# helmholtz-analytics/mpi4torch

Hardware: AMD Instinct MI355X
Metric: allreduce_fwdbwd_algbw_GBps (higher is better)
Workload: dtype bf16; 1 GPU; model=allreduce_1GiB_bf16_fwd_bwd, parallelism=dp1

## Files before the change

csrc/common.hpp:

```cpp
#pragma once

#include <torch/types.h>
#include <c10/util/Exception.h>

#include <cstdint>
#include <string>

namespace m4a {

enum RedOp : int64_t {
  kMax = 0,
  kMin = 1,
  kSum = 2,
  kProd = 3,
  kLAnd = 4,
  kBAnd = 5,
  kLOr = 6,
  kBOr = 7,
  kLXor = 8,
  kBXor = 9,
  kMinLoc = 10,
  kMaxLoc = 11,
};

inline const char* red_op_name(int64_t op) {
  switch (op) {
    case kMax: return "MPI_MAX";
    case kMin: return "MPI_MIN";
    case kSum: return "MPI_SUM";
    case kProd: return "MPI_PROD";
    case kLAnd: return "MPI_LAND";
    case kBAnd: return "MPI_BAND";
    case kLOr: return "MPI_LOR";
    case kBOr: return "MPI_BOR";
    case kLXor: return "MPI_LXOR";
    case kBXor: return "MPI_BXOR";
    case kMinLoc: return "MPI_MINLOC";
    case kMaxLoc: return "MPI_MAXLOC";
    default: return "<invalid op>";
  }
}

struct Config {
  bool force_host_staging = false;
  bool trace_enabled = false;
  bool debug_collectives = false;
  bool force_full_path = false;
  int64_t op_timeout_ms = 0;
  bool force_hierarchical = false;
  int64_t pipeline_chunk_bytes = 256ll << 20;
  enum AllreduceEngine : int { kAllreduceAuto = 0, kAllreduceNative, kAllreduceRccl };
  int allreduce_engine = kAllreduceAuto;
};

Config& config();
void reload_config_from_env();

}
```

csrc/extension.cpp:

```cpp

#include "ops.hpp"
#include "transport.hpp"

#include <torch/script.h>
#include <torch/extension.h>

#include <rccl/rccl.h>

namespace m4a {
namespace {

std::string& world_group_name() {
  static std::string name;
  return name;
}

c10::intrusive_ptr<Communicator> comm_world() {
  return c10::make_intrusive<Communicator>(world_group_name());
}

c10::intrusive_ptr<Communicator> comm_from_group(std::string group_name) {
  return c10::make_intrusive<Communicator>(std::move(group_name));
}

// ... 42 lines not shown
  m.def("JoinDummies", join_dummies_op);
}

}
}

PYBIND11_MODULE(TORCH_EXTENSION_NAME, m) {
  m.doc() = "mpi4torch_amd native core: RCCL-over-xGMI autograd collectives";

  m.def("_set_world_group_name",
        [](const std::string& name) { m4a::world_group_name() = name; });
  m.def("_get_world_group_name",
        []() { return m4a::world_group_name(); });

  m.def("force_host_staging",
        [](bool enabled) { m4a::config().force_host_staging = enabled; });
  m.def("host_staging_forced",
        []() { return m4a::config().force_host_staging; });

  m.def("force_full_path",
        [](bool enabled) { m4a::config().force_full_path = enabled; });

  m.def("_pack_roundtrip", &m4a::debug_pack_roundtrip);
  m.def("_bitwise_reduce", &m4a::debug_bitwise_reduce);
  m.def("_fp8_reduce", &m4a::debug_fp8_reduce);
  m.def("_arith_reduce", &m4a::debug_arith_reduce);
  m.def("_pairloc_reduce", &m4a::debug_pairloc_reduce);
  m.def("_mx8_quantize", &m4a::debug_mx8_quantize);
  m.def("_mx8_reduce", &m4a::debug_mx8_reduce);
  m.def("_mx8_dequantize", &m4a::debug_mx8_dequantize, py::arg("payload"),
        py::arg("scales"), py::arg("numel"), py::arg("dtype"),
        py::arg("out") = c10::optional<at::Tensor>());
  m.def("reload_config", &m4a::reload_config_from_env);

  m.def("_rccl_version", []() {
    int v = 0;
    ncclGetVersion(&v);
    return v;
  });

  m.attr("MPI_MAX") = (int64_t)m4a::kMax;
  m.attr("MPI_MIN") = (int64_t)m4a::kMin;
  m.attr("MPI_SUM") = (int64_t)m4a::kSum;
  m.attr("MPI_PROD") = (int64_t)m4a::kProd;
  m.attr("MPI_LAND") = (int64_t)m4a::kLAnd;
  m.attr("MPI_BAND") = (int64_t)m4a::kBAnd;
  m.attr("MPI_LOR") = (int64_t)m4a::kLOr;
  m.attr("MPI_BOR") = (int64_t)m4a::kBOr;
  m.attr("MPI_LXOR") = (int64_t)m4a::kLXor;
  m.attr("MPI_BXOR") = (int64_t)m4a::kBXor;
  m.attr("MPI_MINLOC") = (int64_t)m4a::kMinLoc;
  m.attr("MPI_MAXLOC") = (int64_t)m4a::kMaxLoc;
}
```

csrc/kernels.hip:

```cpp

#include <hip/hip_runtime.h>
#include <hip/hip_fp8.h>
#include "kernels.hpp"

namespace m4a {

namespace {

struct SlabArgs {
  const char* src;
  char* dst;
  long long row_b;
  long long chunks_per_row;
  long long total_chunks;
  long long src_pitch_b;
  long long dst_pitch_b;
};

template <int N>
struct SlabPack {
  SlabArgs s[N];
};

typedef unsigned int v4u __attribute__((ext_vector_type(4)));
template <typename T>
struct NtVec {
  using type = T;
};
template <>
struct NtVec<uint4> {
  using type = v4u;
};

template <typename VecT, int NSLABS>
__global__ __launch_bounds__(256) void slab_copy_kernel(SlabPack<NSLABS> pack) {
  constexpr long long G = (long long)sizeof(VecT);
  const SlabArgs& a = pack.s[blockIdx.z];
  const long long stride = (long long)gridDim.x * blockDim.x;
  for (long long i = (long long)blockIdx.x * blockDim.x + threadIdx.x;
       i < a.total_chunks; i += stride) {
    const long long b = i / a.chunks_per_row;
    const long long c = i - b * a.chunks_per_row;
    const char* srow = a.src + b * a.src_pitch_b;
    char* drow = a.dst + b * a.dst_pitch_b;
    long long head =
        (G - ((long long)(uintptr_t)drow & (G - 1))) & (G - 1);
    if (head > a.row_b) head = a.row_b;
    const long long body = (a.row_b - head) / G;
    if (c < body) {
      using NT = typename NtVec<VecT>::type;
      const NT* sp = reinterpret_cast<const NT*>(srow + head) + c;
      NT* dp = reinterpret_cast<NT*>(drow + head) + c;
      __builtin_nontemporal_store(__builtin_nontemporal_load(sp), dp);
    } else {
      for (long long k = 0; k < head; ++k) drow[k] = srow[k];
      for (long long k = head + body * G; k < a.row_b; ++k) drow[k] = srow[k];
    }
  }
}

template <typename VecT>
void launch_bucket(const SlabDesc* descs, int n, hipStream_t stream) {
  constexpr long long G = (long long)sizeof(VecT);
  while (n > 0) {
    const int take = n < kMaxSlabsPerLaunch ? n : kMaxSlabsPerLaunch;
    SlabPack<kMaxSlabsPerLaunch> pack{};
    long long max_chunks = 0;
    for (int i = 0; i < take; ++i) {
      const SlabDesc& d = descs[i];
      SlabArgs& a = pack.s[i];
      a.src = static_cast<const char*>(d.src);
      a.dst = static_cast<char*>(d.dst);
      a.row_b = d.count * d.after_b;
      a.src_pitch_b = d.src_pitch_b;
      a.dst_pitch_b = d.dst_pitch_b;
      a.chunks_per_row = (a.row_b >= G ? a.row_b / G : 0) + 1;
      a.total_chunks = d.before * a.chunks_per_row;
      if (a.total_chunks > max_chunks) max_chunks = a.total_chunks;
    }
    for (int i = take; i < kMaxSlabsPerLaunch; ++i) {
      pack.s[i] = pack.s[0];
      pack.s[i].total_chunks = 0;
    }
    if (max_chunks > 0) {
      long long blocks = (max_chunks + 255) / 256;
      if (blocks > 4096) blocks = 4096;
      if (blocks < 1) blocks = 1;
      dim3 grid((unsigned)blocks, 1, (unsigned)take);
      hipLaunchKernelGGL((slab_copy_kernel<VecT, kMaxSlabsPerLaunch>), grid,
                         dim3(256), 0, stream, pack);
    }
    descs += take;
    n -= take;
  }
}


template <int Q>
__device__ inline uint4 byte_window_q(const unsigned int d[8], int rbits) {
  if (rbits == 0) return make_uint4(d[Q], d[Q + 1], d[Q + 2], d[Q + 3]);
  auto take = [&](int j) {
    unsigned long long w =
        ((unsigned long long)d[Q + j + 1] << 32) | d[Q + j];
    return (unsigned int)(w >> rbits);
  };
  return make_uint4(take(0), take(1), take(2), take(3));
}

__device__ inline uint4 byte_window(const uint4& lo, const uint4& hi, int s) {
  const unsigned int d[8] = {lo.x, lo.y, lo.z, lo.w, hi.x, hi.y, hi.z, hi.w};
  const int q = s >> 2;
  const int rbits = (s & 3) * 8;
  switch (q) {
    case 0: return byte_window_q<0>(d, rbits);
    case 1: return byte_window_q<1>(d, rbits);
    case 2: return byte_window_q<2>(d, rbits);
    default: return byte_window_q<3>(d, rbits);
  }
}

template <int NSLABS>
__global__ __launch_bounds__(256) void slab_copy_shift_kernel(
    SlabPack<NSLABS> pack) {
  const SlabArgs& a = pack.s[blockIdx.z];
  const long long stride = (long long)gridDim.x * blockDim.x;
  for (long long i = (long long)blockIdx.x * blockDim.x + threadIdx.x;
       i < a.total_chunks; i += stride) {
    const long long b = i / a.chunks_per_row;
    const long long c = i - b * a.chunks_per_row;
    const char* srow = a.src + b * a.src_pitch_b;
    char* drow = a.dst + b * a.dst_pitch_b;
    long long head = (16 - ((long long)(uintptr_t)drow & 15)) & 15;
    if (head > a.row_b) head = a.row_b;
    const long long body = (a.row_b - head) / 16;
    const char* sbase = srow + head;
    const int s = (int)((uintptr_t)sbase & 15);
    const long long bodyv = (s == 0) ? body : (body > 0 ? body - 1 : 0);
    const long long vs = (s == 0 || s <= head) ? 0 : 1;
    if (c >= vs && c < bodyv) {
      const char* sal = sbase - s + 16 * c;
      if (s == 0) {
        __builtin_nontemporal_store(
            __builtin_nontemporal_load(reinterpret_cast<const v4u*>(sal)),
            reinterpret_cast<v4u*>(drow + head + 16 * c));
      } else {
        const uint4 lo = *reinterpret_cast<const uint4*>(sal);
        const uint4 hi = *reinterpret_cast<const uint4*>(sal + 16);
        const uint4 w = byte_window(lo, hi, s);
        __builtin_nontemporal_store(
            *reinterpret_cast<const v4u*>(&w),
            reinterpret_cast<v4u*>(drow + head + 16 * c));
      }
    } else if (c == bodyv) {
      if (bodyv <= vs) {
        for (long long k = 0; k < a.row_b; ++k) drow[k] = srow[k];
      } else {
        const long long lo_end = head + vs * 16;
        for (long long k = 0; k < lo_end; ++k) drow[k] = srow[k];
        for (long long k = head + bodyv * 16; k < a.row_b; ++k) {
          drow[k] = srow[k];
        }
      }
    }
  }
}

void launch_shift_bucket(const SlabDesc* descs, int n, hipStream_t stream) {
  while (n > 0) {
    const int take = n < kMaxSlabsPerLaunch ? n : kMaxSlabsPerLaunch;
    SlabPack<kMaxSlabsPerLaunch> pack{};
    long long max_chunks = 0;
    for (int i = 0; i < take; ++i) {
      const SlabDesc& d = descs[i];
      SlabArgs& a = pack.s[i];
      a.src = static_cast<const char*>(d.src);
      a.dst = static_cast<char*>(d.dst);
      a.row_b = d.count * d.after_b;
      a.src_pitch_b = d.src_pitch_b;
      a.dst_pitch_b = d.dst_pitch_b;
      a.chunks_per_row = (a.row_b >= 16 ? a.row_b / 16 : 0) + 1;
      a.total_chunks = d.before * a.chunks_per_row;
      if (a.total_chunks > max_chunks) max_chunks = a.total_chunks;
    }
    for (int i = take; i < kMaxSlabsPerLaunch; ++i) {
      pack.s[i] = pack.s[0];
      pack.s[i].total_chunks = 0;
    }
    if (max_chunks > 0) {
      long long blocks = (max_chunks + 255) / 256;
      if (blocks > 4096) blocks = 4096;
      if (blocks < 1) blocks = 1;
      dim3 grid((unsigned)blocks, 1, (unsigned)take);
      hipLaunchKernelGGL((slab_copy_shift_kernel<kMaxSlabsPerLaunch>), grid,
                         dim3(256), 0, stream, pack);
    }
    descs += take;
    n -= take;
  }
}

inline int slab_granule(const SlabDesc& d) {
  const long long delta =
      (long long)((uintptr_t)d.src - (uintptr_t)d.dst);
  const long long pdelta = d.src_pitch_b - d.dst_pitch_b;
  for (int g = 16; g > 1; g >>= 1) {
    if ((delta & (g - 1)) == 0 && (pdelta & (g - 1)) == 0) return g;
  }
  return 1;
}

struct OpAnd {
  __device__ static uint4 apply(uint4 a, uint4 b) {
    return make_uint4(a.x & b.x, a.y & b.y, a.z & b.z, a.w & b.w);
  }
  __device__ static unsigned char apply(unsigned char a, unsigned char b) {
    return a & b;
  }
};
struct OpOr {
  __device__ static uint4 apply(uint4 a, uint4 b) {
    return make_uint4(a.x | b.x, a.y | b.y, a.z | b.z, a.w | b.w);
  }
  __device__ static unsigned char apply(unsigned char a, unsigned char b) {
    return a | b;
  }
};
struct OpXor {
  __device__ static uint4 apply(uint4 a, uint4 b) {
    return make_uint4(a.x ^ b.x, a.y ^ b.y, a.z ^ b.z, a.w ^ b.w);
  }
  __device__ static unsigned char apply(unsigned char a, unsigned char b) {
    return a ^ b;
  }
};

template <typename T, typename Op>
__global__ __launch_bounds__(256) void bitwise_reduce_kernel(
    const T* __restrict__ in, T* __restrict__ out, long long chunk_elems,
    long long nranks) {
  using NT = typename NtVec<T>::type;
  const long long stride = (long long)gridDim.x * blockDim.x;
  for (long long i = (long long)blockIdx.x * blockDim.x + threadIdx.x;
       i < chunk_elems; i += stride) {
    NT av = __builtin_nontemporal_load(reinterpret_cast<const NT*>(in) + i);
    T acc = *reinterpret_cast<const T*>(&av);
    for (long long r = 1; r < nranks; ++r) {
      NT bv = __builtin_nontemporal_load(reinterpret_cast<const NT*>(in) +
                                         r * chunk_elems + i);
      acc = Op::apply(acc, *reinterpret_cast<const T*>(&bv));
    }
    __builtin_nontemporal_store(*reinterpret_cast<const NT*>(&acc),
                                reinterpret_cast<NT*>(out) + i);
  }
}

template <typename T, typename Op>
void launch_bitred(const void* in, void* out, int64_t chunk_elems, int nranks,
                   hipStream_t stream) {
  long long blocks = (chunk_elems + 255) / 256;
  if (blocks > 4096) blocks = 4096;
  if (blocks < 1) blocks = 1;
  hipLaunchKernelGGL((bitwise_reduce_kernel<T, Op>), dim3((unsigned)blocks),
                     dim3(256), 0, stream, static_cast<const T*>(in),
                     static_cast<T*>(out), (long long)chunk_elems,
                     (long long)nranks);
}

}

void launch_slab_copy(const SlabDesc* descs, int n, hipStream_t stream) {
  int i = 0;
  while (i < n) {
    const int g = slab_granule(descs[i]);
    int j = i + 1;
    while (j < n && slab_granule(descs[j]) == g) ++j;
    switch (g) {
      case 16: launch_bucket<uint4>(descs + i, j - i, stream); break;
      case 8: launch_bucket<unsigned long long>(descs + i, j - i, stream); break;
      case 4: launch_bucket<unsigned int>(descs + i, j - i, stream); break;
      default:
        launch_shift_bucket(descs + i, j - i, stream);
        break;
    }
    i = j;
  }
}

void launch_bitwise_reduce(const void* in, void* out, int64_t chunk_bytes,
                           int nranks, int op, hipStream_t stream) {
  const bool vec16 = (chunk_bytes % 16 == 0) &&
                     (reinterpret_cast<uintptr_t>(in) % 16 == 0) &&
                     (reinterpret_cast<uintptr_t>(out) % 16 == 0);
  if (vec16) {
    const int64_t elems = chunk_bytes / 16;
    switch (op) {
// ... 85 lines not shown
    for (int d = 0; d < 4; ++d) {
      unsigned int od = 0;
      for (int k = 0; k < 4; ++k) {
        od |= (unsigned int)f32_to_fp8<E5M2>(acc[4 * d + k]) << (8 * k);
      }
      o[d] = od;
    }
    __builtin_nontemporal_store(o, reinterpret_cast<v4u*>(out) + i);
  }
}

template <typename Op, bool E5M2>
__global__ __launch_bounds__(256) void fp8_reduce_kernel_scalar(
    const unsigned char* __restrict__ in, unsigned char* __restrict__ out,
    long long n, long long nranks) {
  const long long stride = (long long)gridDim.x * blockDim.x;
  for (long long i = (long long)blockIdx.x * blockDim.x + threadIdx.x;
       i < n; i += stride) {
    float acc = fp8_to_f32<E5M2>(in[i]);
    for (long long r = 1; r < nranks; ++r) {
      acc = Op::apply(acc, fp8_to_f32<E5M2>(in[r * n + i]));
    }
    out[i] = f32_to_fp8<E5M2>(acc);
  }
}

template <typename Op, bool E5M2>
void launch_fp8_reduce_t(const void* in, void* out, int64_t n, int nranks,
                         hipStream_t stream) {
  const bool vec = (n % 16 == 0) &&
                   (reinterpret_cast<uintptr_t>(in) % 16 == 0) &&
                   (reinterpret_cast<uintptr_t>(out) % 16 == 0);
  const long long work = vec ? n / 16 : n;
  long long blocks = (work + 255) / 256;
  if (blocks > 4096) blocks = 4096;
  if (blocks < 1) blocks = 1;
  if (vec) {
    hipLaunchKernelGGL((fp8_reduce_kernel<Op, E5M2>), dim3((unsigned)blocks),
                       dim3(256), 0, stream,
                       static_cast<const unsigned char*>(in),
                       static_cast<unsigned char*>(out), (long long)n,
                       (long long)nranks);
  } else {
    hipLaunchKernelGGL((fp8_reduce_kernel_scalar<Op, E5M2>),
                       dim3((unsigned)blocks), dim3(256), 0, stream,
                       static_cast<const unsigned char*>(in),
                       static_cast<unsigned char*>(out), (long long)n,
                       (long long)nranks);
  }
}

}

void launch_fp8_reduce(const void* in, void* out, int64_t n_elems, int nranks,
                       int op, bool e5m2, hipStream_t stream) {
  auto dispatch = [&](auto opv) {
    using Op = decltype(opv);
    if (e5m2) {
      launch_fp8_reduce_t<Op, true>(in, out, n_elems, nranks, stream);
    } else {
      launch_fp8_reduce_t<Op, false>(in, out, n_elems, nranks, stream);
    }
  };
  switch (op) {
    case 0: dispatch(FAdd{}); break;
    case 1: dispatch(FMul{}); break;
    case 2: dispatch(FMin{}); break;
    default: dispatch(FMax{}); break;
  }
}


namespace {

constexpr long long kMaxGrid = 1ll << 30;

struct TF32 {
  using S = float;
  static constexpr int E = 4;
  __device__ static void unpack(v4u w, float* f) {
    for (int d = 0; d < 4; ++d) f[d] = __uint_as_float(w[d]);
  }
  __device__ static v4u pack(const float* f) {
    v4u o;
    for (int d = 0; d < 4; ++d) o[d] = __float_as_uint(f[d]);
    return o;
  }
  __device__ static float ld(const S* p) { return *p; }
  __device__ static void st(S* p, float f) { *p = f; }
};

__device__ inline unsigned int f32_to_bf16_bits(float f) {
  const unsigned int u = __float_as_uint(f);
  if (f != f) return 0x7FC0u;
  return (u + 0x7FFFu + ((u >> 16) & 1u)) >> 16;
}

struct TBF16 {
  using S = unsigned short;
  static constexpr int E = 8;
  __device__ static void unpack(v4u w, float* f) {
    for (int d = 0; d < 4; ++d) {
      f[2 * d] = __uint_as_float(w[d] << 16);
      f[2 * d + 1] = __uint_as_float(w[d] & 0xFFFF0000u);
    }
  }
  __device__ static v4u pack(const float* f) {
    v4u o;
// ... 86 lines not shown
      arith_reduce_scalar_range<T, Op>(own, staged, stride_b, nranks, me, out,
                                       nvec * E, n_elems, 1);
    }
  }
}

template <typename T, typename Op>
__global__ __launch_bounds__(256) void arith_reduce_kernel_scalar(
    const char* __restrict__ own, const char* __restrict__ staged,
    long long stride_b, int nranks, int me, char* __restrict__ out,
    long long n_elems) {
  arith_reduce_scalar_range<T, Op>(
      own, staged, stride_b, nranks, me, out,
      (long long)blockIdx.x * blockDim.x + threadIdx.x, n_elems,
      (long long)gridDim.x * blockDim.x);
}

__global__ __launch_bounds__(256) void arith_reduce_copy_kernel(
    const char* __restrict__ src, char* __restrict__ dst, long long nvec,
    long long nbytes) {
  const long long items = nvec + (nbytes > nvec * 16 ? 1 : 0);
  for (long long t = blockIdx.x; t * 256 < items; t += gridDim.x) {
    const long long i = t * 256 + threadIdx.x;
    if (i < nvec) {
      __builtin_nontemporal_store(
          __builtin_nontemporal_load(reinterpret_cast<const v4u*>(src) + i),
          reinterpret_cast<v4u*>(dst) + i);
    } else if (i == nvec) {
      for (long long k = nvec * 16; k < nbytes; ++k) dst[k] = src[k];
    }
  }
}

inline unsigned arith_grid(long long items) {
  long long blocks = (items + 255) / 256;
  if (blocks > kMaxGrid) blocks = kMaxGrid;
  if (blocks < 1) blocks = 1;
  return (unsigned)blocks;
}

template <typename T, typename Op>
void launch_arith_reduce_t(const void* own, const void* staged,
                           int64_t stride_elems, int nranks, int me,
                           void* out, int64_t n, hipStream_t stream) {
  const long long esize = (long long)sizeof(typename T::S);
  const long long stride_b = (long long)stride_elems * esize;
  auto al16 = [](const void* p) {
    return reinterpret_cast<uintptr_t>(p) % 16 == 0;
  };
  const bool vec = al16(own) && al16(out) && al16(staged) && stride_b % 16 == 0;
  if (vec) {
    const long long nvec = n / T::E;
    const long long items = nvec + (n % T::E ? 1 : 0);
    hipLaunchKernelGGL((arith_reduce_kernel<T, Op>), dim3(arith_grid(items)),
                       dim3(256), 0, stream, static_cast<const char*>(own),
                       static_cast<const char*>(staged), stride_b, nranks, me,
                       static_cast<char*>(out), nvec, (long long)n);
  } else {
    hipLaunchKernelGGL((arith_reduce_kernel_scalar<T, Op>),
                       dim3(arith_grid(n)), dim3(256), 0, stream,
                       static_cast<const char*>(own),
                       static_cast<const char*>(staged), stride_b, nranks, me,
                       static_cast<char*>(out), (long long)n);
  }
}

}

void launch_arith_copy(const void* src, void* dst, int64_t nbytes,
                       hipStream_t stream) {
  if (nbytes <= 0) return;
  if (reinterpret_cast<uintptr_t>(src) % 16 != 0 ||
      reinterpret_cast<uintptr_t>(dst) % 16 != 0) {
    SlabDesc d;
    d.src = src;
    d.dst = dst;
    d.before = 1;
    d.count = 1;
    d.after_b = nbytes;
    d.src_pitch_b = nbytes;
    d.dst_pitch_b = nbytes;
    launch_slab_copy(&d, 1, stream);
    return;
  }
  const long long nvec = nbytes / 16;
  const long long items = nvec + (nbytes % 16 ? 1 : 0);
  hipLaunchKernelGGL(arith_reduce_copy_kernel, dim3(arith_grid(items)),
                     dim3(256), 0, stream, static_cast<const char*>(src),
                     static_cast<char*>(dst), nvec, (long long)nbytes);
}

void launch_arith_reduce(const void* own, const void* staged,
                         int64_t stride_elems, int nranks, int me, void* out,
                         int64_t n_elems, int op, int dtype,
                         hipStream_t stream) {
  if (n_elems <= 0) return;
  if (nranks == 1) {
    launch_arith_copy(own, out, n_elems * (dtype == 0 ? 4 : 2), stream);
    return;
  }
  auto dispatch = [&](auto opv) {
    using Op = decltype(opv);
    switch (dtype) {
      case 0:
        launch_arith_reduce_t<TF32, Op>(own, staged, stride_elems, nranks, me,
                                        out, n_elems, stream);
        break;
      case 1:
        launch_arith_reduce_t<TBF16, Op>(own, staged, stride_elems, nranks, me,
                                         out, n_elems, stream);
        break;
      default:
        launch_arith_reduce_t<TF16, Op>(own, staged, stride_elems, nranks, me,
                                        out, n_elems, stream);
        break;
    }
  };
  switch (op) {
    case 0: dispatch(FAdd{}); break;
    case 1: dispatch(FMul{}); break;
    case 2: dispatch(FMin{}); break;
    default: dispatch(FMax{}); break;
  }
}


#include <hip/hip_fp16.h>
#include <hip/hip_bfloat16.h>

namespace {

// ... 6 lines not shown
template <>
__device__ inline bool pl_lt<hip_bfloat16>(hip_bfloat16 a, hip_bfloat16 b) {
  return (float)a < (float)b;
}
template <typename T>
__device__ inline bool pl_eq(T a, T b) { return !pl_lt(a, b) && !pl_lt(b, a); }

template <typename T, bool MAXLOC>
__global__ __launch_bounds__(256) void pairloc_reduce_kernel(
    const T* __restrict__ in, T* __restrict__ out, long long n,
    long long nranks) {
  const long long stride = (long long)gridDim.x * blockDim.x;
  for (long long i = (long long)blockIdx.x * blockDim.x + threadIdx.x;
       i < n; i += stride) {
    T bv = in[2 * i];
    T bl = in[2 * i + 1];
    for (long long r = 1; r < nranks; ++r) {
      const T v = in[r * 2 * n + 2 * i];
      const T l = in[r * 2 * n + 2 * i + 1];
      const bool better = MAXLOC ? pl_lt(bv, v) : pl_lt(v, bv);
      if (better || (pl_eq(v, bv) && pl_lt(l, bl))) {
        bv = v;
        bl = l;
      }
    }
    out[2 * i] = bv;
    out[2 * i + 1] = bl;
  }
}

template <typename T>
void launch_pairloc_t(const void* in, void* out, int64_t n, int nranks,
                      int op, hipStream_t stream) {
  long long blocks = (n + 255) / 256;
  if (blocks > 4096) blocks = 4096;
  if (blocks < 1) blocks = 1;
  if (op == 0) {
    hipLaunchKernelGGL((pairloc_reduce_kernel<T, false>),
                       dim3((unsigned)blocks), dim3(256), 0, stream,
                       static_cast<const T*>(in), static_cast<T*>(out),
                       (long long)n, (long long)nranks);
  } else {
    hipLaunchKernelGGL((pairloc_reduce_kernel<T, true>),
                       dim3((unsigned)blocks), dim3(256), 0, stream,
                       static_cast<const T*>(in), static_cast<T*>(out),
                       (long long)n, (long long)nranks);
  }
}

}

void launch_pairloc_reduce(const void* in, void* out, int64_t n_pairs,
                           int nranks, int op, int dtype,
                           hipStream_t stream) {
  switch (dtype) {
    case 0: launch_pairloc_t<float>(in, out, n_pairs, nranks, op, stream); break;
    case 1: launch_pairloc_t<double>(in, out, n_pairs, nranks, op, stream); break;
    case 2: launch_pairloc_t<__half>(in, out, n_pairs, nranks, op, stream); break;
    case 3: launch_pairloc_t<hip_bfloat16>(in, out, n_pairs, nranks, op, stream); break;
    case 4: launch_pairloc_t<signed char>(in, out, n_pairs, nranks, op, stream); break;
    case 5: launch_pairloc_t<unsigned char>(in, out, n_pairs, nranks, op, stream); break;
    case 6: launch_pairloc_t<short>(in, out, n_pairs, nranks, op, stream); break;
    case 7: launch_pairloc_t<int>(in, out, n_pairs, nranks, op, stream); break;
    default: launch_pairloc_t<long long>(in, out, n_pairs, nranks, op, stream); break;
  }
}

}
```

csrc/kernels.hpp:

```cpp
#pragma once

#include <hip/hip_runtime_api.h>
#include <cstdint>

namespace m4a {

struct SlabDesc {
  const void* src;
  void* dst;
  int64_t before;
  int64_t count;
  int64_t after_b;
  int64_t src_pitch_b;
  int64_t dst_pitch_b;
};

constexpr int kMaxSlabsPerLaunch = 8;

void launch_slab_copy(const SlabDesc* descs, int n, hipStream_t stream);

void launch_bitwise_reduce(const void* in, void* out, int64_t chunk_bytes,
                           int nranks, int op, hipStream_t stream);

void launch_pairloc_reduce(const void* in, void* out, int64_t n_pairs,
                           int nranks, int op, int dtype, hipStream_t stream);

void launch_fp8_reduce(const void* in, void* out, int64_t n_elems,
                       int nranks, int op, bool e5m2, hipStream_t stream);

void launch_arith_reduce(const void* own, const void* staged,
                         int64_t stride_elems, int nranks, int me, void* out,
                         int64_t n_elems, int op, int dtype,
                         hipStream_t stream);
void launch_arith_copy(const void* src, void* dst, int64_t nbytes,
                       hipStream_t stream);

void launch_mx8_quantize(const void* in, void* payload, void* scales,
                         int64_t n_elems, int dtype, hipStream_t stream);
void launch_mx8_reduce(const void* payload_in, const void* scales_in,
                       void* payload_out, void* scales_out, int64_t n_groups,
                       int nranks, hipStream_t stream);
void launch_mx8_dequantize(const void* payload, const void* scales, void* out,
                           int64_t n_elems, int dtype, hipStream_t stream);

}
```

csrc/mx8_kernels.hip:

```cpp

#include <hip/hip_runtime.h>
#include <hip/hip_fp8.h>
#include "kernels.hpp"

namespace m4a {

namespace {

typedef unsigned int v4u __attribute__((ext_vector_type(4)));
typedef unsigned int v2u __attribute__((ext_vector_type(2)));
typedef unsigned char u8;

constexpr unsigned kInfBits = 0x7f800000u;
constexpr unsigned kQNaNBits = 0x7fc00000u;

enum { kF32 = 0, kBF16 = 1, kF16 = 2 };

template <int K> struct Elem { using type = float; };
template <> struct Elem<kBF16> { using type = unsigned short; };
template <> struct Elem<kF16> { using type = unsigned short; };

__device__ inline float e4m3_to_f32(u8 b) {
  __hip_fp8_e4m3 v;
  v.__x = b;
// ... 336 lines not shown
      w[0] = t[0];
      w[EPL / 4 - 1] = t[1];
    }
    float x[EPL];
    for (int d = 0; d < EPL / 4; ++d) {
      for (int k = 0; k < 4; ++k) {
        x[4 * d + k] = mx8_dequant((u8)(w[d] >> (8 * k)), sb);
      }
    }
    __builtin_nontemporal_store(pack16<K, EPL>(x),
                                reinterpret_cast<v4u*>(out) + i);
  }
  const int tail = (int)(N - nfull * 32);
  if (tail > 0 && blockIdx.x == gridDim.x - 1 && threadIdx.x == 0) {
    dequant_group_scalar<K>(pay + nfull * 32, sc[nfull], tail,
                            reinterpret_cast<T*>(out) + nfull * 32);
  }
}

template <int K>
__global__ __launch_bounds__(256) void mx8_dequantize_kernel_scalar(
    const u8* __restrict__ pay, const u8* __restrict__ sc,
    void* __restrict__ out, long long G, long long N) {
  using T = typename Elem<K>::type;
  const long long stride = (long long)gridDim.x * blockDim.x;
  for (long long g = (long long)blockIdx.x * blockDim.x + threadIdx.x; g < G;
       g += stride) {
    const long long left = N - g * 32;
    dequant_group_scalar<K>(pay + g * 32, sc[g], left < 32 ? (int)left : 32,
                            reinterpret_cast<T*>(out) + g * 32);
  }
}

inline unsigned grid_for(long long work) {
  long long blocks = (work + 255) / 256;
  if (blocks > 4096) blocks = 4096;
  if (blocks < 1) blocks = 1;
  return (unsigned)blocks;
}

inline bool aligned(const void* p, uintptr_t a) {
  return (reinterpret_cast<uintptr_t>(p) & (a - 1)) == 0;
}

template <int K>
void launch_quantize_t(const void* in, void* pay, void* sc, int64_t N,
                       hipStream_t stream) {
  constexpr int LPG = K == kF32 ? 8 : 4;
  const long long G = (N + 31) / 32;
  const long long nfull = N / 32;
  if (aligned(in, 16) && aligned(pay, 32 / LPG)) {
    hipLaunchKernelGGL((mx8_quantize_kernel<K>), dim3(grid_for(nfull * LPG)),
                       dim3(256), 0, stream, in, static_cast<u8*>(pay),
                       static_cast<u8*>(sc), nfull, (long long)N);
  } else {
    hipLaunchKernelGGL((mx8_quantize_kernel_scalar<K>), dim3(grid_for(G)),
                       dim3(256), 0, stream, in, static_cast<u8*>(pay),
                       static_cast<u8*>(sc), G, (long long)N);
  }
}

template <int K>
void launch_dequantize_t(const void* pay, const void* sc, void* out, int64_t N,
                         hipStream_t stream) {
  constexpr int LPG = K == kF32 ? 8 : 4;
  const long long G = (N + 31) / 32;
  const long long nfull = N / 32;
  if (aligned(out, 16) && aligned(pay, 32 / LPG)) {
    hipLaunchKernelGGL((mx8_dequantize_kernel<K>),
                       dim3(grid_for(nfull * LPG)), dim3(256), 0, stream,
                       static_cast<const u8*>(pay),
                       static_cast<const u8*>(sc), out, nfull, (long long)N);
  } else {
    hipLaunchKernelGGL((mx8_dequantize_kernel_scalar<K>), dim3(grid_for(G)),
                       dim3(256), 0, stream, static_cast<const u8*>(pay),
                       static_cast<const u8*>(sc), out, G, (long long)N);
  }
}

}

void launch_mx8_quantize(const void* in, void* payload, void* scales,
                         int64_t n_elems, int dtype, hipStream_t stream) {
  if (n_elems <= 0) return;
  switch (dtype) {
    case 0: launch_quantize_t<kF32>(in, payload, scales, n_elems, stream); break;
    case 1: launch_quantize_t<kBF16>(in, payload, scales, n_elems, stream); break;
    default: launch_quantize_t<kF16>(in, payload, scales, n_elems, stream); break;
  }
}

void launch_mx8_reduce(const void* payload_in, const void* scales_in,
                       void* payload_out, void* scales_out, int64_t n_groups,
                       int nranks, hipStream_t stream) {
  if (n_groups <= 0) return;
  const u8* pin = static_cast<const u8*>(payload_in);
  const u8* sin = static_cast<const u8*>(scales_in);
  u8* pout = static_cast<u8*>(payload_out);
  u8* sout = static_cast<u8*>(scales_out);
  if (aligned(pin, 16) && aligned(pout, 16)) {
    hipLaunchKernelGGL(mx8_reduce_kernel, dim3(grid_for(n_groups * 2)),
                       dim3(256), 0, stream, pin, sin, pout, sout,
                       (long long)n_groups, (long long)nranks);
  } else {
    hipLaunchKernelGGL(mx8_reduce_kernel_scalar, dim3(grid_for(n_groups)),
                       dim3(256), 0, stream, pin, sin, pout, sout,
                       (long long)n_groups, (long long)nranks);
  }
}

void launch_mx8_dequantize(const void* payload, const void* scales, void* out,
                           int64_t n_elems, int dtype, hipStream_t stream) {
  if (n_elems <= 0) return;
  switch (dtype) {
    case 0: launch_dequantize_t<kF32>(payload, scales, out, n_elems, stream); break;
    case 1: launch_dequantize_t<kBF16>(payload, scales, out, n_elems, stream); break;
    default: launch_dequantize_t<kF16>(payload, scales, out, n_elems, stream); break;
  }
}

}
```

csrc/ops.cpp:

```cpp

#include "ops.hpp"
#include "transport.hpp"
#include "kernels.hpp"

#include <torch/csrc/autograd/function.h>
#include <torch/csrc/autograd/functions/utils.h>
#include <torch/csrc/autograd/variable.h>
#include <ATen/core/TensorBody.h>
#include <ATen/WrapDimUtils.h>

#include <ATen/hip/impl/HIPStreamMasqueradingAsCUDA.h>

#include <algorithm>
#include <cstdlib>
#include <cstring>
#include <functional>
#include <limits>
#include <map>
#include <mutex>
#include <tuple>

namespace m4a {

using at::Tensor;
// ... 105 lines not shown
        d.dst_pitch_b = counts[i] * g.after_b;
      } else {
        d.src = bp + row_lo * counts[i] * g.after_b;
        d.src_pitch_b = counts[i] * g.after_b;
        d.dst = base + displs[i] * g.after_b + row_lo * g.axis * g.after_b;
        d.dst_pitch_b = g.axis * g.after_b;
      }
      descs.push_back(d);
    }
    if (!descs.empty()) {
      launch_slab_copy(descs.data(), (int)descs.size(),
                       current_gpu_stream(full));
    }
  } else {
    if (g.before * g.after == 0) return;
    auto f3 = full.view({g.before, g.axis, g.after})
                  .narrow(0, row_lo, rows);
    for (size_t i = 0; i < counts.size(); ++i) {
      if (counts[i] == 0) continue;
      auto b3 = blocks[i].view({g.before, counts[i], g.after})
                    .narrow(0, row_lo, rows);
      if (pack) {
        b3.copy_(f3.narrow(1, displs[i], counts[i]));
      } else {
        f3.narrow(1, displs[i], counts[i]).copy_(b3);
      }
    }
  }
}


Tensor fast_clone(const Tensor& in) {
  if (!in.is_cuda() || in.numel() == 0) return in.clone();
  auto out = at::empty_like(in);
  SlabDesc d;
  d.src = in.data_ptr();
  d.dst = out.data_ptr();
  d.before = 1;
  d.count = 1;
  d.after_b = in.numel() * in.element_size();
  d.src_pitch_b = d.after_b;
  d.dst_pitch_b = d.after_b;
  launch_slab_copy(&d, 1, current_gpu_stream(in));
  return out;
}

std::vector<int64_t> prefix_displs(const std::vector<int64_t>& counts) {
  std::vector<int64_t> d(counts.size(), 0);
  for (size_t i = 1; i < counts.size(); ++i) d[i] = d[i - 1] + counts[i - 1];
  return d;
}

int64_t phase_count(const Tensor& t, int64_t per_rank_bytes) {
  const int64_t c = config().pipeline_chunk_bytes;
  if (c <= 0) return 1;
  if (t.is_cuda()) {
    hipStreamCaptureStatus st = hipStreamCaptureStatusNone;
    (void)hipStreamIsCapturing(current_gpu_stream(t), &st);
    if (st != hipStreamCaptureStatusNone) return 1;
  }
  return std::min<int64_t>(
      4, std::max<int64_t>(1, (per_rank_bytes + c - 1) / c));
}

void phased_funnel_exchange(
    Transport& tr, int64_t K, int64_t rows,
    const std::vector<Tensor>& sblocks, const std::vector<int>& speers,
    const std::vector<int64_t>& srowe, std::vector<Tensor>& rblocks,
    const std::vector<int>& rpeers, const std::vector<int64_t>& rrowe,
    const std::function<void(int64_t, int64_t)>& pack_phase,
    const std::function<void(int64_t, int64_t)>& unpack_phase) {
  auto bound = [&](int64_t k) { return rows * k / K; };
  auto slice = [](const Tensor& blk, int64_t lo, int64_t len) {
    auto flat = blk.view({-1});
    return len > 0 ? flat.narrow(0, lo, len) : flat.narrow(0, 0, 0);
  };
// ... 202 lines not shown

bool arith_float_dtype(at::ScalarType t) {
  return t == at::kFloat || t == at::kBFloat16 || t == at::kHalf;
}

int arith_dtype_code(at::ScalarType t) {
  return t == at::kFloat ? 0 : (t == at::kBFloat16 ? 1 : 2);
}

int arith_op_code(int64_t op) {
  return op == kSum ? 0 : (op == kProd ? 1 : (op == kMin ? 2 : 3));
}

Tensor arith_local_reduce(const std::vector<Tensor>& srcs, int kop,
                          at::ScalarType out_dtype) {
  auto acc = srcs[0].to(at::kFloat);
  for (size_t r = 1; r < srcs.size(); ++r) {
    auto v = srcs[r].to(at::kFloat);
    if (kop == 0) acc = acc + v;
    else if (kop == 1) acc = acc * v;
    else if (kop == 2) acc = at::minimum(acc, v);
    else acc = at::maximum(acc, v);
  }
  return acc.to(out_dtype);
}

Tensor native_allreduce(Transport& tr, const Tensor& in, int64_t op) {
  const int P = tr.size();
  const int me = tr.rank();
  const int64_t N = in.numel();
  auto out = at::empty_like(in);
  if (P == 1) {
    if (in.is_cuda()) {
      launch_arith_copy(in.data_ptr(), out.data_ptr(),
                        N * (int64_t)in.element_size(),
                        current_gpu_stream(in));
    } else {
      out.copy_(in);
    }
    return out;
  }
  TORCH_CHECK(arith_float_dtype(in.scalar_type()) && is_arith(op),
              "native_allreduce reduces bf16/fp16/fp32 with sum/prod/min/max");
  const int kop = arith_op_code(op);
  const int64_t unit = 16 / (int64_t)in.element_size();
  const int64_t nunits = N / unit;
  std::vector<int64_t> counts(P);
  for (int p = 0; p < P; ++p) {
    counts[p] = (nunits / P + (p < nunits % P ? 1 : 0)) * unit;
  }
  counts[P - 1] += N - nunits * unit;
  auto displs = prefix_displs(counts);
  auto flat = in.view({-1});
  auto out_flat = out.view({-1});
  const int64_t mine = counts[me];
  const int64_t slot = (mine + unit - 1) / unit * unit;
  auto staging = at::empty({(int64_t)(P - 1) * slot}, in.options());
  {
    std::vector<Tensor> sends, recvs;
    std::vector<int> speers, rpeers;
    for (int p = 0; p < P; ++p) {
      if (p == me) continue;
      if (counts[p] > 0) {
        sends.push_back(flat.narrow(0, displs[p], counts[p]));
        speers.push_back(p);
      }
      if (mine > 0) {
        recvs.push_back(
            staging.narrow(0, (int64_t)(p - (p > me ? 1 : 0)) * slot, mine));
// ... 1859 lines not shown
```

Baseline: 3173 GB/s.

## Add tiled slab-copy grid planning and size-gated launch grids across kernels

Reworks the slab copy launcher into a planner that chooses a 2D tiled grid (rows on y, 256-chunk tiles on x) when rows are wide, balances tile counts across the slabs in one launch, and uses 32-bit index division when that fits. Grid caps are unified through a stream_grid helper that lifts the fixed 4096-block cap for large outputs and reduction kernels, and accepts a runtime override. fast_clone now uses the flat vectorised copy kernel instead of the slab path. The aim is to cut per-element index arithmetic and grid-stride looping on large copies, in exchange for more launch planning logic and very large grids.

```diff
diff --git a/csrc/common.hpp b/csrc/common.hpp
--- a/csrc/common.hpp
+++ b/csrc/common.hpp
@@ -53,6 +53,8 @@
   int allreduce_engine = kAllreduceAuto;
 };
 
+int64_t set_max_grid(int64_t n);
+
 Config& config();
 void reload_config_from_env();
 
diff --git a/csrc/extension.cpp b/csrc/extension.cpp
--- a/csrc/extension.cpp
+++ b/csrc/extension.cpp
@@ -98,6 +98,7 @@
         py::arg("scales"), py::arg("numel"), py::arg("dtype"),
         py::arg("out") = c10::optional<at::Tensor>());
   m.def("reload_config", &m4a::reload_config_from_env);
+  m.def("_set_max_grid", &m4a::set_max_grid, py::arg("n"));
 
   m.def("_rccl_version", []() {
     int v = 0;
diff --git a/csrc/kernels.hip b/csrc/kernels.hip
--- a/csrc/kernels.hip
+++ b/csrc/kernels.hip
@@ -1,11 +1,22 @@
 
 #include <hip/hip_runtime.h>
 #include <hip/hip_fp8.h>
+#include <atomic>
 #include "kernels.hpp"
 
 namespace m4a {
 
 namespace {
+std::atomic<int64_t> g_max_grid{0};
+}
+
+int64_t set_max_grid(int64_t n) { return g_max_grid.exchange(n > 0 ? n : 0); }
+int64_t max_grid_setting() { return g_max_grid.load(std::memory_order_relaxed); }
+
+namespace {
+
+constexpr long long kFp8ReduceGrid = kMaxGrid;
+constexpr long long kArithReduceGrid = kMaxGrid;
 
 struct SlabArgs {
   const char* src;
@@ -15,6 +26,8 @@
   long long total_chunks;
   long long src_pitch_b;
   long long dst_pitch_b;
+  long long before;
+  long long tiles_per_row;
 };
 
 template <int N>
@@ -32,15 +45,37 @@
   using type = v4u;
 };
 
-template <typename VecT, int NSLABS>
+template <bool TILED, typename F>
+__device__ inline void slab_for_each_chunk(const SlabArgs& a, F&& f) {
+  if (TILED) {
+    for (long long b = blockIdx.y; b < a.before; b += gridDim.y) {
+      for (long long t = blockIdx.x; t < a.tiles_per_row; t += gridDim.x) {
+        const long long c = t * 256 + threadIdx.x;
+        if (c < a.chunks_per_row) f(b, c);
+      }
+    }
+  } else {
+    const bool narrow = a.total_chunks <= 0xffffffffll;
+    for (long long t = blockIdx.x; t * 256 < a.total_chunks; t += gridDim.x) {
+      const long long i = t * 256 + threadIdx.x;
+      if (i >= a.total_chunks) continue;
+      if (narrow) {
+        const unsigned int q = (unsigned int)i / (unsigned int)a.chunks_per_row;
+        f((long long)q,
+          (long long)((unsigned int)i - q * (unsigned int)a.chunks_per_row));
+      } else {
+        const long long b = i / a.chunks_per_row;
+        f(b, i - b * a.chunks_per_row);
+      }
+    }
+  }
+}
+
+template <typename VecT, int NSLABS, bool TILED>
 __global__ __launch_bounds__(256) void slab_copy_kernel(SlabPack<NSLABS> pack) {
   constexpr long long G = (long long)sizeof(VecT);
   const SlabArgs& a = pack.s[blockIdx.z];
-  const long long stride = (long long)gridDim.x * blockDim.x;
-  for (long long i = (long long)blockIdx.x * blockDim.x + threadIdx.x;
-       i < a.total_chunks; i += stride) {
-    const long long b = i / a.chunks_per_row;
-    const long long c = i - b * a.chunks_per_row;
+  slab_for_each_chunk<TILED>(a, [&](long long b, long long c) {
     const char* srow = a.src + b * a.src_pitch_b;
     char* drow = a.dst + b * a.dst_pitch_b;
     long long head =
@@ -56,39 +91,106 @@
       for (long long k = 0; k < head; ++k) drow[k] = srow[k];
       for (long long k = head + body * G; k < a.row_b; ++k) drow[k] = srow[k];
     }
-  }
+  });
+}
+
+struct SlabLaunch {
+  SlabPack<kMaxSlabsPerLaunch> pack;
+  dim3 grid;
+  bool tiled;
+  bool any;
+};
+
+constexpr long long kSmallLaunch = 4096;
+inline long long balanced_tiles(long long max_tiles, long long sum_tiles,
+                                int take, long long per_x) {
+  if (max_tiles * per_x <= kSmallLaunch) return max_tiles;
+  const long long mean = (sum_tiles + take - 1) / take;
+  const long long floor_x = (kSmallLaunch + per_x - 1) / per_x;
+  const long long x = mean > floor_x ? mean : floor_x;
+  return x < max_tiles ? x : max_tiles;
+}
+
+inline SlabLaunch plan_slab_launch(const SlabDesc* descs, int take,
+                                   long long G, bool worker) {
+  SlabLaunch L{};
+  long long max_chunks = 0, max_tiles_per_row = 0, max_before = 0;
+  long long sum_flat_tiles = 0, sum_tiles_per_row = 0;
+  bool tiled = true;
+  for (int i = 0; i < take; ++i) {
+    const SlabDesc& d = descs[i];
+    SlabArgs& a = L.pack.s[i];
+    a.src = static_cast<const char*>(d.src);
+    a.dst = static_cast<char*>(d.dst);
+    a.row_b = d.count * d.after_b;
+    a.src_pitch_b = d.src_pitch_b;
+    a.dst_pitch_b = d.dst_pitch_b;
+    a.before = d.before;
+    const bool exact =
+        !worker && a.row_b > 0 && a.row_b % G == 0 &&
+        reinterpret_cast<uintptr_t>(d.dst) % (uintptr_t)G == 0 &&
+        (d.before <= 1 || d.dst_pitch_b % G == 0);
+    a.chunks_per_row = (a.row_b >= G ? a.row_b / G : 0) + (exact ? 0 : 1);
+    a.total_chunks = d.before * a.chunks_per_row;
+    a.tiles_per_row = (a.chunks_per_row + 255) / 256;
+    if (a.total_chunks <= 0) {
+      a.total_chunks = 0;
+      a.before = 0;
+      continue;
+    }
+    if (a.chunks_per_row < 256 ||
+        (a.tiles_per_row * 256 - a.chunks_per_row) * 16 > a.chunks_per_row) {
+      tiled = false;
+    }
+    if (a.total_chunks > max_chunks) max_chunks = a.total_chunks;
+    sum_flat_tiles += (a.total_chunks + 255) / 256;
+    sum_tiles_per_row += a.tiles_per_row;
+    if (a.tiles_per_row > max_tiles_per_row) max_tiles_per_row = a.tiles_per_row;
+    if (a.before > max_before) max_before = a.before;
+  }
+  for (int i = take; i < kMaxSlabsPerLaunch; ++i) {
+    L.pack.s[i] = L.pack.s[0];
+    L.pack.s[i].total_chunks = 0;
+    L.pack.s[i].before = 0;
+  }
+  L.any = max_chunks > 0;
+  if (worker || G < 16) {
+    L.tiled = false;
+    L.grid = dim3(stream_grid((max_chunks + 255) / 256, kCappedGrid), 1,
+                  (unsigned)take);
+    return L;
+  }
+  L.tiled = tiled;
+  if (tiled) {
+    const long long ylim = max_before < 65535 ? max_before : 65535;
+    const unsigned gy = stream_grid(ylim, 65535);
+    L.grid = dim3(stream_grid(balanced_tiles(max_tiles_per_row, sum_tiles_per_row,
+                                             take, (long long)gy * take),
+                              kMaxGrid),
+                  gy, (unsigned)take);
+  } else {
+    L.grid = dim3(stream_grid(balanced_tiles((max_chunks + 255) / 256,
+                                             sum_flat_tiles, take, take),
+                              kMaxGrid),
+                  1, (unsigned)take);
+  }
+  return L;
 }
 
 template <typename VecT>
 void launch_bucket(const SlabDesc* descs, int n, hipStream_t stream) {
-  constexpr long long G = (long long)sizeof(VecT);
   while (n > 0) {
     const int take = n < kMaxSlabsPerLaunch ? n : kMaxSlabsPerLaunch;
-    SlabPack<kMaxSlabsPerLaunch> pack{};
-    long long max_chunks = 0;
-    for (int i = 0; i < take; ++i) {
-      const SlabDesc& d = descs[i];
-      SlabArgs& a = pack.s[i];
-      a.src = static_cast<const char*>(d.src);
-      a.dst = static_cast<char*>(d.dst);
-      a.row_b = d.count * d.after_b;
-      a.src_pitch_b = d.src_pitch_b;
-      a.dst_pitch_b = d.dst_pitch_b;
-      a.chunks_per_row = (a.row_b >= G ? a.row_b / G : 0) + 1;
-      a.total_chunks = d.before * a.chunks_per_row;
-      if (a.total_chunks > max_chunks) max_chunks = a.total_chunks;
-    }
-    for (int i = take; i < kMaxSlabsPerLaunch; ++i) {
-      pack.s[i] = pack.s[0];
-      pack.s[i].total_chunks = 0;
-    }
-    if (max_chunks > 0) {
-      long long blocks = (max_chunks + 255) / 256;
-      if (blocks > 4096) blocks = 4096;
-      if (blocks < 1) blocks = 1;
-      dim3 grid((unsigned)blocks, 1, (unsigned)take);
-      hipLaunchKernelGGL((slab_copy_kernel<VecT, kMaxSlabsPerLaunch>), grid,
-                         dim3(256), 0, stream, pack);
+    const SlabLaunch L =
+        plan_slab_launch(descs, take, (long long)sizeof(VecT), false);
+    if (L.any) {
+      if (L.tiled) {
+        hipLaunchKernelGGL((slab_copy_kernel<VecT, kMaxSlabsPerLaunch, true>),
+                           L.grid, dim3(256), 0, stream, L.pack);
+      } else {
+        hipLaunchKernelGGL((slab_copy_kernel<VecT, kMaxSlabsPerLaunch, false>),
+                           L.grid, dim3(256), 0, stream, L.pack);
+      }
     }
     descs += take;
     n -= take;
@@ -123,11 +225,7 @@
 __global__ __launch_bounds__(256) void slab_copy_shift_kernel(
     SlabPack<NSLABS> pack) {
   const SlabArgs& a = pack.s[blockIdx.z];
-  const long long stride = (long long)gridDim.x * blockDim.x;
-  for (long long i = (long long)blockIdx.x * blockDim.x + threadIdx.x;
-       i < a.total_chunks; i += stride) {
-    const long long b = i / a.chunks_per_row;
-    const long long c = i - b * a.chunks_per_row;
+  slab_for_each_chunk<false>(a, [&](long long b, long long c) {
     const char* srow = a.src + b * a.src_pitch_b;
     char* drow = a.dst + b * a.dst_pitch_b;
     long long head = (16 - ((long long)(uintptr_t)drow & 15)) & 15;
@@ -162,37 +260,16 @@
         }
       }
     }
-  }
+  });
 }
 
 void launch_shift_bucket(const SlabDesc* descs, int n, hipStream_t stream) {
   while (n > 0) {
     const int take = n < kMaxSlabsPerLaunch ? n : kMaxSlabsPerLaunch;
-    SlabPack<kMaxSlabsPerLaunch> pack{};
-    long long max_chunks = 0;
-    for (int i = 0; i < take; ++i) {
-      const SlabDesc& d = descs[i];
-      SlabArgs& a = pack.s[i];
-      a.src = static_cast<const char*>(d.src);
-      a.dst = static_cast<char*>(d.dst);
-      a.row_b = d.count * d.after_b;
-      a.src_pitch_b = d.src_pitch_b;
-      a.dst_pitch_b = d.dst_pitch_b;
-      a.chunks_per_row = (a.row_b >= 16 ? a.row_b / 16 : 0) + 1;
-      a.total_chunks = d.before * a.chunks_per_row;
-      if (a.total_chunks > max_chunks) max_chunks = a.total_chunks;
-    }
-    for (int i = take; i < kMaxSlabsPerLaunch; ++i) {
-      pack.s[i] = pack.s[0];
-      pack.s[i].total_chunks = 0;
-    }
-    if (max_chunks > 0) {
-      long long blocks = (max_chunks + 255) / 256;
-      if (blocks > 4096) blocks = 4096;
-      if (blocks < 1) blocks = 1;
-      dim3 grid((unsigned)blocks, 1, (unsigned)take);
-      hipLaunchKernelGGL((slab_copy_shift_kernel<kMaxSlabsPerLaunch>), grid,
-                         dim3(256), 0, stream, pack);
+    const SlabLaunch L = plan_slab_launch(descs, take, 16, true);
+    if (L.any) {
+      hipLaunchKernelGGL((slab_copy_shift_kernel<kMaxSlabsPerLaunch>), L.grid,
+                         dim3(256), 0, stream, L.pack);
     }
     descs += take;
     n -= take;
@@ -257,10 +334,10 @@
 template <typename T, typename Op>
 void launch_bitred(const void* in, void* out, int64_t chunk_elems, int nranks,
                    hipStream_t stream) {
-  long long blocks = (chunk_elems + 255) / 256;
-  if (blocks > 4096) blocks = 4096;
-  if (blocks < 1) blocks = 1;
-  hipLaunchKernelGGL((bitwise_reduce_kernel<T, Op>), dim3((unsigned)blocks),
+  const unsigned blocks =
+      stream_grid((chunk_elems + 255) / 256,
+                  size_gated_grid((long long)chunk_elems * (long long)sizeof(T)));
+  hipLaunchKernelGGL((bitwise_reduce_kernel<T, Op>), dim3(blocks),
                      dim3(256), 0, stream, static_cast<const T*>(in),
                      static_cast<T*>(out), (long long)chunk_elems,
                      (long long)nranks);
@@ -412,18 +489,16 @@
                    (reinterpret_cast<uintptr_t>(in) % 16 == 0) &&
                    (reinterpret_cast<uintptr_t>(out) % 16 == 0);
   const long long work = vec ? n / 16 : n;
-  long long blocks = (work + 255) / 256;
-  if (blocks > 4096) blocks = 4096;
-  if (blocks < 1) blocks = 1;
+  const unsigned blocks = stream_grid((work + 255) / 256, kFp8ReduceGrid);
   if (vec) {
-    hipLaunchKernelGGL((fp8_reduce_kernel<Op, E5M2>), dim3((unsigned)blocks),
+    hipLaunchKernelGGL((fp8_reduce_kernel<Op, E5M2>), dim3(blocks),
                        dim3(256), 0, stream,
                        static_cast<const unsigned char*>(in),
                        static_cast<unsigned char*>(out), (long long)n,
                        (long long)nranks);
   } else {
     hipLaunchKernelGGL((fp8_reduce_kernel_scalar<Op, E5M2>),
-                       dim3((unsigned)blocks), dim3(256), 0, stream,
+                       dim3(blocks), dim3(256), 0, stream,
                        static_cast<const unsigned char*>(in),
                        static_cast<unsigned char*>(out), (long long)n,
                        (long long)nranks);
@@ -452,8 +527,6 @@
 
 
 namespace {
-
-constexpr long long kMaxGrid = 1ll << 30;
 
 struct TF32 {
   using S = float;
@@ -606,11 +679,8 @@
   }
 }
 
-inline unsigned arith_grid(long long items) {
-  long long blocks = (items + 255) / 256;
-  if (blocks > kMaxGrid) blocks = kMaxGrid;
-  if (blocks < 1) blocks = 1;
-  return (unsigned)blocks;
+inline unsigned arith_grid(long long items, long long cap) {
+  return stream_grid((items + 255) / 256, cap);
 }
 
 template <typename T, typename Op>
@@ -626,13 +696,13 @@
   if (vec) {
     const long long nvec = n / T::E;
     const long long items = nvec + (n % T::E ? 1 : 0);
-    hipLaunchKernelGGL((arith_reduce_kernel<T, Op>), dim3(arith_grid(items)),
+    hipLaunchKernelGGL((arith_reduce_kernel<T, Op>), dim3(arith_grid(items, kArithReduceGrid)),
                        dim3(256), 0, stream, static_cast<const char*>(own),
                        static_cast<const char*>(staged), stride_b, nranks, me,
                        static_cast<char*>(out), nvec, (long long)n);
   } else {
     hipLaunchKernelGGL((arith_reduce_kernel_scalar<T, Op>),
-                       dim3(arith_grid(n)), dim3(256), 0, stream,
+                       dim3(arith_grid(n, kArithReduceGrid)), dim3(256), 0, stream,
                        static_cast<const char*>(own),
                        static_cast<const char*>(staged), stride_b, nranks, me,
                        static_cast<char*>(out), (long long)n);
@@ -641,8 +711,8 @@
 
 }
 
-void launch_arith_copy(const void* src, void* dst, int64_t nbytes,
-                       hipStream_t stream) {
+void launch_flat_copy(const void* src, void* dst, int64_t nbytes,
+                      hipStream_t stream) {
   if (nbytes <= 0) return;
   if (reinterpret_cast<uintptr_t>(src) % 16 != 0 ||
       reinterpret_cast<uintptr_t>(dst) % 16 != 0) {
@@ -659,7 +729,8 @@
   }
   const long long nvec = nbytes / 16;
   const long long items = nvec + (nbytes % 16 ? 1 : 0);
-  hipLaunchKernelGGL(arith_reduce_copy_kernel, dim3(arith_grid(items)),
+  hipLaunchKernelGGL(arith_reduce_copy_kernel,
+                     dim3(arith_grid(items, kMaxGrid)),
                      dim3(256), 0, stream, static_cast<const char*>(src),
                      static_cast<char*>(dst), nvec, (long long)nbytes);
 }
@@ -670,7 +741,7 @@
                          hipStream_t stream) {
   if (n_elems <= 0) return;
   if (nranks == 1) {
-    launch_arith_copy(own, out, n_elems * (dtype == 0 ? 4 : 2), stream);
+    launch_flat_copy(own, out, n_elems * (dtype == 0 ? 4 : 2), stream);
     return;
   }
   auto dispatch = [&](auto opv) {
@@ -743,17 +814,17 @@
 template <typename T>
 void launch_pairloc_t(const void* in, void* out, int64_t n, int nranks,
                       int op, hipStream_t stream) {
-  long long blocks = (n + 255) / 256;
-  if (blocks > 4096) blocks = 4096;
-  if (blocks < 1) blocks = 1;
+  const unsigned blocks =
+      stream_grid((n + 255) / 256,
+                  size_gated_grid((long long)n * 2 * (long long)sizeof(T)));
   if (op == 0) {
     hipLaunchKernelGGL((pairloc_reduce_kernel<T, false>),
-                       dim3((unsigned)blocks), dim3(256), 0, stream,
+                       dim3(blocks), dim3(256), 0, stream,
                        static_cast<const T*>(in), static_cast<T*>(out),
                        (long long)n, (long long)nranks);
   } else {
     hipLaunchKernelGGL((pairloc_reduce_kernel<T, true>),
-                       dim3((unsigned)blocks), dim3(256), 0, stream,
+                       dim3(blocks), dim3(256), 0, stream,
                        static_cast<const T*>(in), static_cast<T*>(out),
                        (long long)n, (long long)nranks);
   }
diff --git a/csrc/kernels.hpp b/csrc/kernels.hpp
--- a/csrc/kernels.hpp
+++ b/csrc/kernels.hpp
@@ -14,6 +14,25 @@
   int64_t src_pitch_b;
   int64_t dst_pitch_b;
 };
+
+constexpr long long kMaxGrid = 1ll << 30;
+constexpr long long kCappedGrid = 4096;
+constexpr long long kLargeOutputBytes = 256ll << 20;
+inline long long size_gated_grid(long long out_bytes) {
+  return out_bytes >= kLargeOutputBytes ? kMaxGrid : kCappedGrid;
+}
+
+int64_t set_max_grid(int64_t n);
+int64_t max_grid_setting();
+
+inline unsigned stream_grid(long long tiles, long long cap) {
+  const long long forced = (long long)max_grid_setting();
+  long long lim = forced > 0 ? forced : cap;
+  if (lim > kMaxGrid) lim = kMaxGrid;
+  long long blocks = tiles < lim ? tiles : lim;
+  if (blocks < 1) blocks = 1;
+  return (unsigned)blocks;
+}
 
 constexpr int kMaxSlabsPerLaunch = 8;
 
@@ -32,8 +51,8 @@
                          int64_t stride_elems, int nranks, int me, void* out,
                          int64_t n_elems, int op, int dtype,
                          hipStream_t stream);
-void launch_arith_copy(const void* src, void* dst, int64_t nbytes,
-                       hipStream_t stream);
+void launch_flat_copy(const void* src, void* dst, int64_t nbytes,
+                      hipStream_t stream);
 
 void launch_mx8_quantize(const void* in, void* payload, void* scales,
                          int64_t n_elems, int dtype, hipStream_t stream);
diff --git a/csrc/mx8_kernels.hip b/csrc/mx8_kernels.hip
--- a/csrc/mx8_kernels.hip
+++ b/csrc/mx8_kernels.hip
@@ -392,11 +392,11 @@
   }
 }
 
-inline unsigned grid_for(long long work) {
-  long long blocks = (work + 255) / 256;
-  if (blocks > 4096) blocks = 4096;
-  if (blocks < 1) blocks = 1;
-  return (unsigned)blocks;
+constexpr long long kQuantizeGrid = kCappedGrid;
+constexpr long long kReduceGrid = kMaxGrid;
+
+inline unsigned grid_for(long long work, long long cap) {
+  return stream_grid((work + 255) / 256, cap);
 }
 
 inline bool aligned(const void* p, uintptr_t a) {
@@ -410,11 +410,13 @@
   const long long G = (N + 31) / 32;
   const long long nfull = N / 32;
   if (aligned(in, 16) && aligned(pay, 32 / LPG)) {
-    hipLaunchKernelGGL((mx8_quantize_kernel<K>), dim3(grid_for(nfull * LPG)),
-                       dim3(256), 0, stream, in, static_cast<u8*>(pay),
+    hipLaunchKernelGGL((mx8_quantize_kernel<K>),
+                       dim3(grid_for(nfull * LPG, kQuantizeGrid)), dim3(256),
+                       0, stream, in, static_cast<u8*>(pay),
                        static_cast<u8*>(sc), nfull, (long long)N);
   } else {
-    hipLaunchKernelGGL((mx8_quantize_kernel_scalar<K>), dim3(grid_for(G)),
+    hipLaunchKernelGGL((mx8_quantize_kernel_scalar<K>),
+                       dim3(grid_for(G, kQuantizeGrid)),
                        dim3(256), 0, stream, in, static_cast<u8*>(pay),
                        static_cast<u8*>(sc), G, (long long)N);
   }
@@ -426,13 +428,16 @@
   constexpr int LPG = K == kF32 ? 8 : 4;
   const long long G = (N + 31) / 32;
   const long long nfull = N / 32;
+  const long long dq_cap = size_gated_grid(
+      (long long)N * (long long)sizeof(typename Elem<K>::type));
   if (aligned(out, 16) && aligned(pay, 32 / LPG)) {
     hipLaunchKernelGGL((mx8_dequantize_kernel<K>),
-                       dim3(grid_for(nfull * LPG)), dim3(256), 0, stream,
-                       static_cast<const u8*>(pay),
+                       dim3(grid_for(nfull * LPG, dq_cap)), dim3(256),
+                       0, stream, static_cast<const u8*>(pay),
                        static_cast<const u8*>(sc), out, nfull, (long long)N);
   } else {
-    hipLaunchKernelGGL((mx8_dequantize_kernel_scalar<K>), dim3(grid_for(G)),
+    hipLaunchKernelGGL((mx8_dequantize_kernel_scalar<K>),
+                       dim3(grid_for(G, dq_cap)),
                        dim3(256), 0, stream, static_cast<const u8*>(pay),
                        static_cast<const u8*>(sc), out, G, (long long)N);
   }
@@ -459,11 +464,13 @@
   u8* pout = static_cast<u8*>(payload_out);
   u8* sout = static_cast<u8*>(scales_out);
   if (aligned(pin, 16) && aligned(pout, 16)) {
-    hipLaunchKernelGGL(mx8_reduce_kernel, dim3(grid_for(n_groups * 2)),
+    hipLaunchKernelGGL(mx8_reduce_kernel,
+                       dim3(grid_for(n_groups * 2, kReduceGrid)),
                        dim3(256), 0, stream, pin, sin, pout, sout,
                        (long long)n_groups, (long long)nranks);
   } else {
-    hipLaunchKernelGGL(mx8_reduce_kernel_scalar, dim3(grid_for(n_groups)),
+    hipLaunchKernelGGL(mx8_reduce_kernel_scalar,
+                       dim3(grid_for(n_groups, kReduceGrid)),
                        dim3(256), 0, stream, pin, sin, pout, sout,
                        (long long)n_groups, (long long)nranks);
   }
diff --git a/csrc/ops.cpp b/csrc/ops.cpp
--- a/csrc/ops.cpp
+++ b/csrc/ops.cpp
@@ -161,16 +161,11 @@
 
 Tensor fast_clone(const Tensor& in) {
   if (!in.is_cuda() || in.numel() == 0) return in.clone();
-  auto out = at::empty_like(in);
-  SlabDesc d;
-  d.src = in.data_ptr();
-  d.dst = out.data_ptr();
-  d.before = 1;
-  d.count = 1;
-  d.after_b = in.numel() * in.element_size();
-  d.src_pitch_b = d.after_b;
-  d.dst_pitch_b = d.after_b;
-  launch_slab_copy(&d, 1, current_gpu_stream(in));
+  TORCH_CHECK(in.is_contiguous(), "fast_clone expects a contiguous tensor");
+  auto out = at::empty_like(in, at::MemoryFormat::Contiguous);
+  launch_flat_copy(in.data_ptr(), out.data_ptr(),
+                   in.numel() * (int64_t)in.element_size(),
+                   current_gpu_stream(in));
   return out;
 }
 
@@ -439,9 +434,9 @@
   auto out = at::empty_like(in);
   if (P == 1) {
     if (in.is_cuda()) {
-      launch_arith_copy(in.data_ptr(), out.data_ptr(),
-                        N * (int64_t)in.element_size(),
-                        current_gpu_stream(in));
+      launch_flat_copy(in.data_ptr(), out.data_ptr(),
+                       N * (int64_t)in.element_size(),
+                       current_gpu_stream(in));
     } else {
       out.copy_(in);
     }
```

Result: no change. 3174 GB/s (median of 3 runs) (+0.0%).
